# bempt/uda_aerial_semantic_segmentation_research

Measured on AMD Instinct MI355X. Metric: training images/sec at 512x512, higher is better.
Workload: dtype fp32

## Files before the change

include/udaseg.h:

```cpp
#ifndef UDASEG_H
#define UDASEG_H

#include <stddef.h>
#include <stdint.h>

#ifdef __cplusplus
extern "C" {
#endif

#define UDASEG_OK 0
#define UDASEG_E_BADARG (-1)
#define UDASEG_E_UNSUPPORTED (-2)
#define UDASEG_E_WORKSPACE (-3)
#define UDASEG_E_HIP (-4)

#define UDASEG_ACT_NONE 0
#define UDASEG_ACT_LEAKY 1

int udaseg_version(void);
#define UDASEG_OPT_GENERIC_GATHER 0
#define UDASEG_OPT_F32_SPLIT 1
#define UDASEG_OPT_WGRAD_GENERIC 2
#define UDASEG_OPT_F32_HALO 3
#define UDASEG_OPT_F3_CFG 4
#define UDASEG_OPT_F3_WS 5
#define UDASEG_OPT_F3_SIGNS 6
#define UDASEG_OPT_IGEMM_TILE 7
#define UDASEG_OPT_IGEMM_X3 8
#define UDASEG_OPT_NO_FOLD 9
#define UDASEG_OPT_WGRAD_X3_BLOCKS 10
#define UDASEG_OPT_WGRAD_BLOCKS 11
#define UDASEG_OPT_WGRAD_NO_XCD 12
#define UDASEG_OPT_WGRAD_X3 13
#define UDASEG_OPT_NO_WGRAD_HALO 14
#define UDASEG_OPT_WGRAD_F3_BLOCKS 15
#define UDASEG_OPT_WGRAD_HALO_BLOCKS 16
#define UDASEG_OPT_WGRAD_DEEP_BLOCKS 17
#define UDASEG_OPT_WGRAD_DB 18
#define UDASEG_OPT_REDUCE_BLOCKS 19
#define UDASEG_OPT_BN_APPLY_PT 20
#define UDASEG_OPT_GEMM_1X1_TILE 21
#define UDASEG_OPT_GEMM_1X1 22
#define UDASEG_OPT_GEMM_1X1_MAXM 23
#define UDASEG_OPT_NO_STREAM 24
#define UDASEG_OPT_HALO_CFG 25
#define UDASEG_OPT_NO_HALO 26
#define UDASEG_OPT_NO_HALO_S2 27
#define UDASEG_OPT_HALO_W16 28
#define UDASEG_OPT_HALO_DEEP 29
#define UDASEG_OPT_HALO_S2_CK 30
#define UDASEG_OPT_UP_CFG 31
#define UDASEG_OPT_WGRAD_UP_BLOCKS 32
#define UDASEG_OPT_COUNT 33
int udaseg_set_option(int key, int value);
int udaseg_get_option(int key);
int udaseg_option_count(void);
const char* udaseg_option_name(int key);
int udaseg_option_epoch(void);
const char* udaseg_last_error(void);
int udaseg_device_count(void);
int udaseg_memset_async(void* ptr, int value, size_t bytes, void* stream);
int udaseg_stream_wait(void* waiter_stream, void* signal_stream);

typedef struct {
  int n, hi, wi, ci;
  int ho, wo, co;
  int kh, kw, stride, pad;
} udaseg_conv_desc;


int udaseg_conv2d_fwd(const udaseg_conv_desc* d, const float* x, const float* w, const float* bias, float* y,
                      int act, float slope, int accumulate, void* stream);
int udaseg_conv2d_fwd_bnstats(const udaseg_conv_desc* d, const float* x, const float* w, const float* bias, float* y,
                              double* stats, void* stream);
int udaseg_conv2d_fwd_fused(const udaseg_conv_desc* d, const float* x, const float* w, const float* bias,
                            const float* residual, float* y, int act, float slope, void* stream);
int udaseg_conv2d_fwd_bf16(const udaseg_conv_desc* d, const void* x, const void* w, const float* bias, const void* residual,
                           void* y, int out_f32, int act, float slope, double* stats, void* stream);
int udaseg_conv2d_dgrad_bf16(const udaseg_conv_desc* d, const void* dy, const void* w_t, void* dx, int accumulate,
                             void* stream);
int udaseg_conv2d_wgrad_bf16(const udaseg_conv_desc* d, const void* x, const void* dy, float* dw, int accumulate, void* stream);
int udaseg_conv2d_dgrad(const udaseg_conv_desc* d, const float* dy, const float* w_t, float* dx, int accumulate,
                        void* stream);
int udaseg_conv2d_dgrad_bnreduce_ok(const udaseg_conv_desc* d);
int udaseg_conv2d_dgrad_bnreduce(const udaseg_conv_desc* d, const float* dy, const float* w_t, float* dx, const float* prev_y,
                                 const float* save_mean, const float* save_rstd, const float* gamma, const float* beta, int act,
                                 float slope, double* bsums, void* stream);
int udaseg_conv2d_dgrad_bnreduce_bf16_ok(const udaseg_conv_desc* d);
int udaseg_conv2d_dgrad_bnreduce_bf16(const udaseg_conv_desc* d, const void* dy, const void* w_t, void* dx, const void* prev_y,
                                      const float* save_mean, const float* save_rstd, const float* gamma, const float* beta,
                                      int act, float slope, double* bsums, void* stream);
int udaseg_conv2d_wgrad(const udaseg_conv_desc* d, const float* x, const float* dy, float* dw, int accumulate,
                        void* stream);
int udaseg_conv2d_fwd_upcat(const udaseg_conv_desc* d, const float* a, const float* skip, int ca, const float* w,
                            const float* bias, float* y, int act, float slope, double* stats, void* stream);
int udaseg_conv2d_fwd_upcat_bf16(const udaseg_conv_desc* d, const void* a, const void* skip, int ca, const void* w,
                                 const float* bias, void* y, int act, float slope, double* stats, void* stream);
int udaseg_conv2d_dgrad_split(const udaseg_conv_desc* d, const float* dy, const float* w_t, float* dx_a, float* dx_b, int ca,
                              void* stream);
int udaseg_conv2d_dgrad_split_bf16(const udaseg_conv_desc* d, const void* dy, const void* w_t, void* dx_a, void* dx_b, int ca,
                                   void* stream);
int udaseg_conv2d_wgrad_part(const udaseg_conv_desc* d, const float* src, int src_c, int c_off, int up, const float* dy,
                             float* dw, int accumulate, void* stream);
int udaseg_conv2d_wgrad_part_bf16(const udaseg_conv_desc* d, const void* src, int src_c, int c_off, int up, const void* dy,
                                  float* dw, int accumulate, void* stream);
int udaseg_pack_dgrad_weights(const udaseg_conv_desc* d, const float* w, float* w_t, void* stream);
int udaseg_pack_dgrad_batched(const float* arena, float* packed, const int* table, int entries, void* stream);
double udaseg_conv_flops(const udaseg_conv_desc* d);

int udaseg_nchw_to_nhwc(const float* x, float* y, int n, int c, int h, int w, int cpad, void* stream);

int udaseg_bn_replicas(void);
int udaseg_bn_stats(const float* y, int64_t pixels, int c, double* sums, void* stream);
int udaseg_bn_stats_bf16(const void* y, int64_t pixels, int c, double* sums, void* stream);
int udaseg_bn_apply(const float* y, const double* sums, const float* gamma, const float* beta, const float* residual,
                    float* z, int64_t pixels, int c, float eps, float momentum, float* running_mean,
                    float* running_var, float* save_mean, float* save_rstd, int act, float slope, void* stream);
int udaseg_bn_apply_eval(const float* y, const float* gamma, const float* beta, const float* running_mean,
                         const float* running_var, const float* residual, float* z, int64_t pixels, int c, float eps,
                         int act, float slope, void* stream);
int udaseg_bn_fold(const float* w, const float* bias, const float* gamma, const float* beta, const float* running_mean,
                   const float* running_var, float eps, int co, int row_len, float* w_folded, float* bias_folded, void* stream);
int udaseg_bn_bwd_reduce(const float* dz, const float* z, const float* y, const float* save_mean,
                         const float* save_rstd, const float* gamma, const float* beta, int64_t pixels, int c,
                         double* bsums, int act, float slope, void* stream);
int udaseg_bn_bwd_apply(const float* dz, const float* z, const float* y, const float* save_mean,
                        const float* save_rstd, const float* gamma, const float* beta, const double* bsums, float* dy,
                        float* dres, float* dgamma, float* dbeta, int64_t pixels, int c, int act, float slope,
                        int accumulate_dy, int accumulate_dres, int accumulate_param, void* stream);
int udaseg_act_bwd(const float* dz, const float* z, float* dy, int64_t count, int act, float slope, void* stream);
int udaseg_channel_sum(const float* x, int64_t pixels, int c, float* out,
                       int accumulate, void* stream);
int udaseg_channel_sum_ws(const float* x, int64_t pixels, int c, float* out, int accumulate, float* scratch,
                          size_t scratch_bytes, void* stream);
size_t udaseg_channel_sum_scratch_bytes(int c);

// ... 197 lines not shown
```

uda_aerial_semantic_segmentation_research_amd/_lib.py:

```python
import ctypes as C
import os

_HERE = os.path.dirname(os.path.abspath(__file__))
LIB_PATH = os.environ.get("UDASEG_LIB", os.path.join(_HERE, "libudaseg_hip.so"))

ACT_NONE = 0
ACT_LEAKY = 1


class ConvDesc(C.Structure):
    _fields_ = [(k, C.c_int) for k in ("n", "hi", "wi", "ci", "ho", "wo", "co", "kh", "kw", "stride", "pad")]


_P = C.c_void_p
_I = C.c_int
_L = C.c_int64
_F = C.c_float
_D = C.POINTER(ConvDesc)

SIGNATURES = {
    "udaseg_version": (_I, []),
    "udaseg_set_option": (_I, [_I, _I]),
    "udaseg_get_option": (_I, [_I]),
    "udaseg_option_count": (_I, []),
# ... 62 lines not shown
    "udaseg_predict_threshold": (_I, [_P, _I, _I, _I, _I, _P, _P]),
    "udaseg_dice_bwd": (_I, [_P, _P, _P, _P, _F, _I, _L, _I, _I, _P, _I, _P]),
    "udaseg_focal_fwd": (_I, [_P, _P, _P, _F, _F, _L, _I, _I, _I, _P, _P, _I, _P]),
    "udaseg_focal_bwd": (_I, [_P, _P, _P, _F, _F, _P, _F, _L, _I, _I, _P, _I, _P]),
    "udaseg_consistency_fwd": (_I, [_P, _P, _F, _I, _L, _I, _I, _P, _P, _P]),
    "udaseg_consistency_bwd": (_I, [_P, _P, _F, _P, _F, _I, _L, _I, _I, _P, _P, _I, _P]),
    "udaseg_argmax_confusion": (_I, [_P, _P, _L, _I, _I, _P, _P, _P]),
    "udaseg_gap_splits": (_I, [_I]),
    "udaseg_gap_linear_sigmoid_fwd": (_I, [_P, _P, _P, _P, _P, _P, _I, _I, _I, _P]),
    "udaseg_gap_linear_sigmoid_bwd": (_I, [_P, _P, _P, _P, _P, _P, _P, _I, _I, _I, _I, _P]),
    "udaseg_bce_logits_fwd": (_I, [_P, _I, _F, _F, _P, _I, _P]),
    "udaseg_bce_logits_bwd": (_I, [_P, _I, _F, _F, _P, _P, _I, _P]),
    "udaseg_adam_flat": (_I, [_P, _P, _P, _P, _L, _F, _F, _F, _F, _F, _F, _P]),
    "udaseg_bn_apply_bf16": (_I, [_P, _P, _P, _P, _P, _P, _L, _I, _F, _F, _P, _P, _P, _P, _I, _F, _P]),
    "udaseg_bn_bwd_reduce_bf16": (_I, [_P, _P, _P, _P, _P, _L, _I, _P, _I, _F, _P]),
    "udaseg_bn_bwd_apply_bf16": (_I, [_P, _P, _P, _P, _P, _P, _P, _P, _P, _P, _P, _L, _I, _I, _F, _I, _I, _I, _P]),
    "udaseg_act_bwd_bf16": (_I, [_P, _P, _P, _L, _I, _F, _P]),
    "udaseg_channel_sum_bf16": (_I, [_P, _L, _I, _P, _I, _P]),
    "udaseg_channel_sum_bf16_ws": (_I, [_P, _L, _I, _P, _I, _P, C.c_size_t, _P]),
    "udaseg_nchw_to_nhwc_bf16": (_I, [_P, _P, _I, _I, _I, _I, _I, _P]),
    "udaseg_cast_f32_to_bf16": (_I, [_P, _P, _L, _P]),
    "udaseg_maxpool3x3s2_fwd_bf16": (_I, [_P, _P, _P, _I, _I, _I, _I, _P]),
    "udaseg_maxpool3x3s2_bwd_bf16": (_I, [_P, _P, _P, _I, _I, _I, _I, _I, _P]),
    "udaseg_upsample2x_concat_bwd_bf16": (_I, [_P, _P, _P, _I, _I, _I, _I, _I, _I, _I, _P]),
    "udaseg_gap_partial_bf16": (_I, [_P, _P, _I, _I, _I, _P]),
    "udaseg_gap_finish": (_I, [_P, _P, _P, _P, _P, _I, _I, _I, _P]),
    "udaseg_gap_bwd_broadcast_bf16": (_I, [_P, _P, _P, _P, _I, _I, _I, _P]),
    "udaseg_gap_bwd_param": (_I, [_P, _P, _P, _P, _P, _I, _I, _I, _P]),
    "udaseg_pack_dgrad_batched_bf16": (_I, [_P, _P, _P, _I, _P]),
    "udaseg_bn_finalize": (_I, [_P, _P, _P, _L, _I, _F, _F, _P, _P, _P, _P, _P, _P, _P]),
    "udaseg_bn_bwd_apply_recompute_bf16": (_I, [_P, _P, _P, _P, _P, _P, _P, _P, _P, _P, _P, _L, _I, _I, _F, _P]),
    "udaseg_conv2d_wgrad_halo_bf16_ok": (_I, [_D, _I]),
    "udaseg_conv2d_wgrad_halo_bf16": (_I, [_D, _P, _P, _I, _P, _P, _P]),
    "udaseg_conv2d_wgrad_bnin_bf16": (_I, [_D, _P, _P, _P, _I, _F, _P, _P, _I, _P]),
    "udaseg_frag_elems": (_L, [_I, _I, _I]),
    "udaseg_set_stats_scratch": (_I, [_P, C.c_size_t]),
    "udaseg_pack_frag_batched_bf16": (_I, [_P, _P, _P, _P, _I, _P]),
    "udaseg_conv_frag_ok": (_I, [_D, _I, _I]),
    "udaseg_conv_frag_preferred": (_I, [_D, _I, _I]),
    "udaseg_conv2d_fwd_frag_bf16": (_I, [_D, _P, _P, _I, _P, _P, _P, _P, _I, _F, _P, _I, _I, _F, _P, _P]),
    "udaseg_conv2d_dgrad_frag_bf16": (_I, [_D, _P, _P, _P, _P, _I, _P, _P, _P, _P, _P, _I, _F, _P, _I, _P]),
    "udaseg_pack_frag_batched_f32x3": (_I, [_P, _P, _P, _P, _I, _P]),
    "udaseg_conv2d_wgrad_halo_f32x3_ok": (_I, [_D, _I]),
    "udaseg_conv2d_wgrad_halo_f32x3": (_I, [_D, _P, _P, _I, _P, _P, _P]),
    "udaseg_conv_f32x3_ok": (_I, [_D, _I, _I]),
    "udaseg_f32x3_force_config": (_I, [_I]),
    "udaseg_conv_f32x3_preferred": (_I, [_D, _I, _I]),
    "udaseg_conv2d_fwd_f32x3": (_I, [_D, _P, _P, _I, _P, _P, _P, _I, _F, _P, _P]),
    "udaseg_conv2d_fwd_f32x3_bnin_ok": (_I, [_D, _I]),
    "udaseg_conv2d_fwd_f32x3_bnin_writes": (_I, [_D]),
    "udaseg_conv2d_fwd_f32x3_bnin": (_I, [_D, _P, _I, _P, _P, _I, _F, _P, _P, _P, _P, _I, _F, _P, _P]),
    "udaseg_conv2d_wgrad_bnin_ok": (_I, [_D, _I]),
    "udaseg_conv2d_wgrad_bnin": (_I, [_D, _P, _I, _P, _P, _I, _F, _P, _P, _I, _P]),
    "udaseg_conv2d_dgrad_f32x3": (_I, [_D, _P, _P, _P, _P, _I, _P, _P, _P, _P, _P, _I, _F, _P, _I, _P]),
    "udaseg_conv_up_f32x3_ok": (_I, [_D, _I]),
    "udaseg_pack_up_batched_f32x3": (_I, [_P, _P, _P, _P, _I, _P]),
    "udaseg_conv2d_fwd_up_f32x3": (_I, [_D, _P, _I, _P, _P, _I, _P, _P]),
    "udaseg_conv2d_dgrad_up_f32x3": (_I, [_D, _P, _I, _P, _P, _P, _P, _P, _P, _P, _I, _F, _P, _I, _P]),
    "udaseg_up_f32x3_force_config": (_I, [_I]),
    "udaseg_conv2d_wgrad_up_f32x3_ok": (_I, [_D, _I]),
    "udaseg_conv2d_wgrad_up_f32x3": (_I, [_D, _P, _I, _P, _P, _P]),
    "udaseg_conv2d_wgrad_halo_slice_f32x3": (_I, [_D, _P, _P, _P, _I, _I, _P]),
    "udaseg_wgrad_up_set_blocks": (_I, [_I]),
    "udaseg_conv_stem_f32x3_ok": (_I, [_D]),
    "udaseg_conv2d_fwd_stem_f32x3": (_I, [_D, _P, _P, _P, _P, _P]),
    "udaseg_conv_n16_f32x3_ok": (_I, [_D, _I]),
    "udaseg_conv2d_fwd_n16_f32x3": (_I, [_D, _P, _P, _P, _I, _F, _P, _P, _P, _P]),
    "udaseg_conv2d_dgrad_n16_f32x3": (_I, [_D, _P, _P, _P, _P, _P, _P, _P, _P, _I, _F, _P, _P]),
    "udaseg_set_workspace": (_I, [_P, C.c_size_t]),
    "udaseg_workspace_bytes": (C.c_size_t, [_D]),
    "udaseg_debug_set_timeline": (_I, [_P, _I]),
    "udaseg_fill_f32": (_I, [_P, _L, _F, _P]),
    "udaseg_axpy_f32": (_I, [_P, _P, _L, _F, _P]),
    "udaseg_add_i64": (_I, [_P, _L, _L, _P]),
    "udaseg_prof_enable": (_I, [_I]),
    "udaseg_prof_reset": (_I, []),
    "udaseg_prof_read": (_I, [_I, C.POINTER(C.c_double), C.POINTER(C.c_double), C.POINTER(C.c_int64)]),
    "udaseg_prof_kernel_count": (_I, []),
    "udaseg_prof_kernel_name": (C.c_char_p, [_I]),
    "udaseg_prof_kernel_read": (_I, [_I, C.POINTER(C.c_double), C.POINTER(C.c_double), C.POINTER(C.c_int64)]),
    "udaseg_prof_records": (_I, [_I, _I, C.POINTER(C.c_double), C.POINTER(C.c_double), C.POINTER(C.c_int), C.POINTER(C.c_int)]),
}

OPTIONS = {"GENERIC_GATHER": 0, "F32_SPLIT": 1, "WGRAD_GENERIC": 2, "F32_HALO": 3, "F3_CFG": 4, "F3_WS": 5, "F3_SIGNS": 6, "IGEMM_TILE": 7, "IGEMM_X3": 8, "NO_FOLD": 9, "WGRAD_X3_BLOCKS": 10, "WGRAD_BLOCKS": 11, "WGRAD_NO_XCD": 12, "WGRAD_X3": 13, "NO_WGRAD_HALO": 14, "WGRAD_F3_BLOCKS": 15, "WGRAD_HALO_BLOCKS": 16, "WGRAD_DEEP_BLOCKS": 17, "WGRAD_DB": 18, "REDUCE_BLOCKS": 19, "BN_APPLY_PT": 20, "GEMM_1X1_TILE": 21, "GEMM_1X1": 22, "GEMM_1X1_MAXM": 23, "NO_STREAM": 24, "HALO_CFG": 25, "NO_HALO": 26, "NO_HALO_S2": 27, "HALO_W16": 28, "HALO_DEEP": 29, "HALO_S2_CK": 30, "UP_CFG": 31, "WGRAD_UP_BLOCKS": 32}

_lib = None


def load():
    global _lib
    if _lib is not None:
        return _lib
    if not os.path.exists(LIB_PATH):
        raise RuntimeError(
            f"{LIB_PATH} not found: the HIP extension is not built. Run `python -c \"import __graft_entry__ as g; "
            f"g.build()\"` (or `make -C {os.path.join(_HERE, 'csrc')}`). There is no CPU fallback.")
    lib = C.CDLL(LIB_PATH)
    for name, (res, args) in SIGNATURES.items():
        fn = getattr(lib, name)
        fn.restype = res
        fn.argtypes = args
    _lib = lib
    return lib


def check(rc, what=""):
    if rc != 0:
        msg = load().udaseg_last_error().decode(errors="replace")
        raise RuntimeError(f"libudaseg_hip {what} failed (rc={rc}): {msg}")


def require_gpu():
    lib = load()
    if lib.udaseg_device_count() < 1:
        raise RuntimeError("libudaseg_hip: no HIP device visible; this path has no CPU fallback")
    return lib
```

uda_aerial_semantic_segmentation_research_amd/csrc/api.hip:

```cpp
#include <string.h>
#include <mutex>
#include <vector>

#include "common.h"
#include "options.h"

namespace udaseg {

static thread_local char g_err[512] = "";

void set_error(const char* fmt, ...) {
  va_list ap;
  va_start(ap, fmt);
  vsnprintf(g_err, sizeof(g_err), fmt, ap);
  va_end(ap);
}

int hip_fail(hipError_t e, const char* what) {
  set_error("%s: %s", what, hipGetErrorString(e));
  return UDASEG_E_HIP;
}

struct ProfRec {
  hipEvent_t a, b;
// ... 161 lines not shown
    }
    g_krecs[k].clear();
  }
  return UDASEG_OK;
}

extern "C" int udaseg_prof_read(int family, double* total_ms, double* total_flops, int64_t* launches) {
  UDASEG_CHECK_ARG(family >= 0 && family < 2 && total_ms && total_flops && launches, "prof_read: bad arguments");
  double ms = 0.0, fl = 0.0;
  for (auto& r : g_recs[family]) {
    hipError_t e = hipEventSynchronize(r.b);
    if (e != hipSuccess) return hip_fail(e, "hipEventSynchronize(prof)");
    float t = 0.f;
    e = hipEventElapsedTime(&t, r.a, r.b);
    if (e != hipSuccess) return hip_fail(e, "hipEventElapsedTime(prof)");
    ms += t;
    fl += r.flops;
  }
  *total_ms = ms;
  *total_flops = fl;
  *launches = (int64_t)g_recs[family].size();
  return UDASEG_OK;
}

extern "C" int udaseg_prof_records(int family, int max_records, double* ms, double* flops, int* kind, int* desc11) {
  UDASEG_CHECK_ARG(family >= 0 && family < 2 && ms && flops && kind && desc11 && max_records >= 0, "prof_records: bad arguments");
  int n = 0;
  for (auto& r : g_recs[family]) {
    if (n >= max_records) break;
    hipError_t e = hipEventSynchronize(r.b);
    if (e != hipSuccess) return hip_fail(e, "hipEventSynchronize(prof)");
    float t = 0.f;
    e = hipEventElapsedTime(&t, r.a, r.b);
    if (e != hipSuccess) return hip_fail(e, "hipEventElapsedTime(prof)");
    ms[n] = t;
    flops[n] = r.flops;
    kind[n] = r.kind;
    const int v[11] = {r.d.n, r.d.hi, r.d.wi, r.d.ci, r.d.ho, r.d.wo, r.d.co, r.d.kh, r.d.kw, r.d.stride, r.d.pad};
    for (int i = 0; i < 11; ++i) desc11[n * 11 + i] = v[i];
    ++n;
  }
  return n;
}

namespace udaseg {
enum { K_INT, K_FLAG, K_OFF0 };
struct OptRow {
  const char* env;
  int kind, dflt;
};
static const OptRow g_opt_rows[UDASEG_OPT_COUNT] = {
     {"UDASEG_IGEMM_GENERIC", K_INT, 0},
     {"UDASEG_F32_SPLIT", K_OFF0, 1},
     {"UDASEG_WGRAD_GENERIC", K_INT, 0},
     {"UDASEG_F32_SPLIT", K_OFF0, 1},
     {"UDASEG_F3_CFG", K_INT, 0},
     {"UDASEG_F3_WS", K_OFF0, 1},
     {"UDASEG_F3_SIGNS", K_OFF0, 1},
     {"UDASEG_IGEMM_TILE", K_INT, 0},
     {"UDASEG_IGEMM_X3", K_INT, 1},
     {"UDASEG_NO_FOLD", K_FLAG, 0},
     {"UDASEG_WGRAD_X3_BLOCKS", K_INT, 1024},
     {"UDASEG_WGRAD_BLOCKS", K_INT, 0},
     {"UDASEG_WGRAD_NO_XCD", K_FLAG, 0},
     {"UDASEG_WGRAD_X3", K_OFF0, 1},
     {"UDASEG_NO_WGRAD_HALO", K_FLAG, 0},
     {"UDASEG_WGRAD_F3_BLOCKS", K_INT, 120},
     {"UDASEG_WGRAD_HALO_BLOCKS", K_INT, 96},
     {"UDASEG_WGRAD_DEEP_BLOCKS", K_INT, 0},
     {"UDASEG_WGRAD_DB", K_INT, 1},
     {"UDASEG_REDUCE_BLOCKS", K_INT, 0},
     {"UDASEG_BN_APPLY_PT", K_INT, 4},
     {"UDASEG_GEMM_1X1_TILE", K_INT, 0},
     {"UDASEG_GEMM_1X1", K_OFF0, 1},
     {"UDASEG_GEMM_1X1_MAXM", K_INT, 73728},
     {"UDASEG_NO_STREAM", K_FLAG, 0},
     {"UDASEG_HALO_CFG", K_INT, 0},
     {"UDASEG_NO_HALO", K_FLAG, 0},
     {"UDASEG_NO_HALO_S2", K_FLAG, 0},
     {"UDASEG_HALO_W16", K_INT, 6},
     {"UDASEG_HALO_DEEP", K_OFF0, 1},
     {"UDASEG_HALO_S2_CK", K_INT, 64},
     {"UDASEG_UP_CFG", K_INT, 0},
     {"UDASEG_WGRAD_UP_BLOCKS", K_INT, 0}};
int g_opt_val[UDASEG_OPT_COUNT];
static int g_opt_default[UDASEG_OPT_COUNT];
std::atomic<bool> g_opt_ready{false};
static std::atomic<int> g_opt_epoch{0};
static std::mutex g_opt_mutex;
void opt_init() {
  std::lock_guard<std::mutex> lk(g_opt_mutex);
  if (g_opt_ready.load(std::memory_order_relaxed)) return;
  for (int k = 0; k < UDASEG_OPT_COUNT; ++k) {
    const OptRow& r = g_opt_rows[k];
    const char* e = getenv(r.env);
    int v = r.dflt;
    if (r.kind == K_INT) v = e ? atoi(e) : r.dflt;
    else if (r.kind == K_FLAG) v = e != nullptr ? 1 : 0;
    else v = (e && atoi(e) == 0) ? 0 : 1;
    g_opt_default[k] = g_opt_val[k] = v;
  }
  g_opt_ready.store(true, std::memory_order_release);
}
}

extern "C" int udaseg_set_option(int key, int value) {
  UDASEG_CHECK_ARG(key >= 0 && key < UDASEG_OPT_COUNT, "set_option: unknown key %d (0 .. %d)", key, UDASEG_OPT_COUNT - 1);
  UDASEG_CHECK_ARG(value >= -1, "set_option: value must be >= 0, or -1 for the default");
  udaseg::opt_get(key);
  std::lock_guard<std::mutex> lk(udaseg::g_opt_mutex);
  udaseg::g_opt_val[key] = value < 0 ? udaseg::g_opt_default[key] : value;
  if (key == UDASEG_OPT_GENERIC_GATHER)
    udaseg::g_opt_val[UDASEG_OPT_WGRAD_GENERIC] = value < 0 ? udaseg::g_opt_default[UDASEG_OPT_WGRAD_GENERIC] : value;
  udaseg::g_opt_epoch.fetch_add(1);
  return UDASEG_OK;
}

extern "C" int udaseg_get_option(int key) {
  if (key < 0 || key >= UDASEG_OPT_COUNT) return -1;
  return udaseg::opt_get(key);
}

extern "C" int udaseg_option_count(void) { return UDASEG_OPT_COUNT; }
extern "C" const char* udaseg_option_name(int key) { return key >= 0 && key < UDASEG_OPT_COUNT ? udaseg::g_opt_rows[key].env : ""; }
extern "C" int udaseg_option_epoch(void) { return udaseg::g_opt_epoch.load(); }

extern "C" int udaseg_prof_kernel_count(void) { return g_nkernels; }
extern "C" const char* udaseg_prof_kernel_name(int kid) { return kname(kid); }

extern "C" int udaseg_prof_kernel_read(int kid, double* total_ms, double* total_flops, int64_t* launches) {
  UDASEG_CHECK_ARG(kid >= 0 && kid < g_nkernels && total_ms && total_flops && launches, "prof_kernel_read: bad arguments");
  double ms = 0.0, fl = 0.0;
  for (auto& r : g_krecs[kid]) {
    hipError_t e = hipEventSynchronize(r.b);
    if (e != hipSuccess) return hip_fail(e, "hipEventSynchronize(kprof)");
    float t = 0.f;
    e = hipEventElapsedTime(&t, r.a, r.b);
    if (e != hipSuccess) return hip_fail(e, "hipEventElapsedTime(kprof)");
    ms += t;
    fl += r.flops;
  }
  *total_ms = ms;
  *total_flops = fl;
  *launches = (int64_t)g_krecs[kid].size();
  return UDASEG_OK;
}
```

uda_aerial_semantic_segmentation_research_amd/csrc/common.h:

```cpp
#pragma once
#include <stdlib.h>
#include <hip/hip_runtime.h>
#include <stdint.h>
#include <stdio.h>
#include <stdarg.h>
#include <atomic>

#include "../../include/udaseg.h"
#include "options.h"

namespace udaseg {

void set_error(const char* fmt, ...);
int hip_fail(hipError_t e, const char* what);

#define UDASEG_CHECK_ARG(cond, ...)                 \
  do {                                              \
    if (!(cond)) {                                  \
      ::udaseg::set_error(__VA_ARGS__);             \
      return UDASEG_E_BADARG;                       \
    }                                               \
  } while (0)

#define UDASEG_LAUNCH_CHECK(what)                          \
// ... 80 lines not shown
      if (o < co && c < ci) v = *reinterpret_cast<const f32x4*>(w + ((size_t)o * T + t) * ci + c);
#pragma unroll
      for (int k = 0; k < 4; ++k) tile[row][4 * q + k] = v[k];
    }
    __syncthreads();
    {
      const int c = 32 * b + row, o = 32 * a + 4 * q;
      if (c < ci && o < co) {
        OutT* dst = wt + ((size_t)c * T + t) * co + o;
        if constexpr (sizeof(OutT) == 4) {
          f32x4 v;
#pragma unroll
          for (int k = 0; k < 4; ++k) v[k] = tile[4 * q + k][row];
          *reinterpret_cast<f32x4*>(dst) = v;
        } else {
          unsigned short h[4];
#pragma unroll
          for (int k = 0; k < 4; ++k) h[k] = __builtin_bit_cast(unsigned short, (__bf16)tile[4 * q + k][row]);
          uint2 pk;
          pk.x = (unsigned)h[0] | ((unsigned)h[1] << 16);
          pk.y = (unsigned)h[2] | ((unsigned)h[3] << 16);
          *reinterpret_cast<uint2*>(dst) = pk;
        }
      }
    }
    __syncthreads();
  }
}
constexpr int PACK_DGRAD_GRID_X = 256;

void* workspace_ptr(size_t* bytes);

constexpr int CHSUM_REPLICAS = 16;
constexpr int CHSUM_DIRECT_BLOCKS = 32;
static __global__ void fold_replicas_kernel(const float* __restrict__ rep, int c, float* __restrict__ out, int accumulate) {
  const int i = blockIdx.x * blockDim.x + threadIdx.x;
  if (i >= c) return;
  float s = 0.f;
#pragma unroll
  for (int r = 0; r < CHSUM_REPLICAS; ++r) s += rep[(size_t)r * c + i];
  out[i] = accumulate ? out[i] + s : s;
}

struct StreamShape {
  int bs;
  int grid;
  int c4;
};

static inline StreamShape stream_shape(int64_t n4, int c4, int max_blocks = 2048, int per_thread = 4) {
  StreamShape s;
  s.c4 = c4;
  int unit;
  if (c4 <= 256) {
    s.bs = (256 / c4) * c4;
    unit = 1;
  } else {
    s.bs = 256;
    unit = (c4 + 255) / 256;
    while ((unit * 256) % c4 != 0) ++unit;
  }
  int64_t want = (n4 + (int64_t)s.bs * per_thread - 1) / ((int64_t)s.bs * per_thread);
  if (want > max_blocks) want = max_blocks;
  if (want < 1) want = 1;
  s.grid = (int)(((want + unit - 1) / unit) * unit);
  while ((int64_t)s.grid * s.bs < c4) s.grid += unit;
  return s;
}


static inline int apply_per_thread() {
  const int v = opt_get(UDASEG_OPT_BN_APPLY_PT);
  return (v < 1 || v > 256) ? 4 : v;
}

bool small_conv_applicable(int k, int stride, int pad, int ci_gather, int co_out);
int launch_small_conv(const float* x, const float* w, const float* bias, float* y, int n, int h, int wd, int ci, int co,
                      int flip, int accumulate, int act, float slope, double* stats, const float* residual, hipStream_t s,
                      int up = 0);
bool small_wgrad_applicable(int k, int stride, int pad, int ci, int co, int ntiles);
int launch_small_wgrad(const float* x, const float* dy, float* dw, int n, int h, int wd, int ci, int co, int accumulate,
                       hipStream_t s, int up = 0, const float* in_scale = nullptr, const float* in_shift = nullptr,
                       int in_act = 0, float in_slope = 0.f);

constexpr int PROF_NKERNELS = 24;
int kprof_id(const char* rocprof_symbol);
hipEvent_t kprof_begin(hipStream_t s);
void kprof_end(int kid, hipEvent_t a, hipStream_t s, double flops);
struct KTimer {
  std::atomic<int>* kid;
  hipStream_t s;
  hipEvent_t ev;
  double work;
  KTimer(std::atomic<int>* k, const char* rocprof_symbol, hipStream_t st, double w) : kid(k), s(st), work(w) {
    if (*kid < 0) *kid = kprof_id(rocprof_symbol);
    ev = kprof_begin(s);
  }
  ~KTimer() { kprof_end(*kid, ev, s, work); }
};
void prof_begin(int family, hipStream_t s);
void prof_suspend(int on);
void prof_end(int family, hipStream_t s, double flops, int kind, const udaseg_conv_desc* d);

}
```

uda_aerial_semantic_segmentation_research_amd/csrc/conv_small.hip:

```cpp
#include "common.h"

namespace udaseg {

constexpr int ST = 16;
constexpr int SH = ST + 2;

constexpr int MAX_DEVICES = 16;
static void* g_workspace[MAX_DEVICES] = {};
static size_t g_workspace_bytes[MAX_DEVICES] = {};
static int current_device() {
  int dev = 0;
  if (hipGetDevice(&dev) != hipSuccess || dev < 0 || dev >= MAX_DEVICES) return -1;
  return dev;
}

struct SmallArgs {
  const float* x;
  const float* w;
  const float* bias;
  float* y;
  int n, h, wd, ci, co;
  const float* residual;
  double* stats;
  int flip;
// ... 370 lines not shown
__global__ void small_wgrad_fold_kernel(const float* __restrict__ partial, int nblocks, int cop, int cip, int co, int ci,
                                        float* __restrict__ dw) {
  const int out = cop * 9 * cip;
  const int idx = blockIdx.x * blockDim.x + threadIdx.x;
  if (idx >= out) return;
  const int c = idx % cip, t = (idx / cip) % 9, o = idx / (cip * 9);
  if (c >= ci || o >= co) return;
  const int per = (nblocks + gridDim.y - 1) / gridDim.y;
  const int b0 = blockIdx.y * per, b1 = min(nblocks, b0 + per);
  float s[8] = {0.f, 0.f, 0.f, 0.f, 0.f, 0.f, 0.f, 0.f};
  int b = b0;
  for (; b + 8 <= b1; b += 8) {
#pragma unroll
    for (int u = 0; u < 8; ++u) s[u] += partial[(size_t)(b + u) * out + idx];
  }
  for (; b < b1; ++b) s[0] += partial[(size_t)b * out + idx];
  const float tot = ((s[0] + s[1]) + (s[2] + s[3])) + ((s[4] + s[5]) + (s[6] + s[7]));
  if (b1 > b0) atomicAdd(dw + ((size_t)o * 9 + t) * ci + c, tot);
}

static int small_grid(int ntiles, int blocks_per_cu) {
  int g = 256 * blocks_per_cu;
  return ntiles < g ? ntiles : g;
}

bool small_conv_applicable(int k, int stride, int pad, int ci_gather, int co_out) {
  if (k != 3 || stride != 1 || pad != 1) return false;
  const int G = (ci_gather + 15) / 16, T = (co_out + 15) / 16;
  return G * T <= 2;
}

int launch_small_conv(const float* x, const float* w, const float* bias, float* y, int n, int h, int wd, int ci, int co,
                      int flip, int accumulate, int act, float slope, double* stats, const float* residual, hipStream_t s,
                      int up) {
  SmallArgs a = {};
  a.up = up;
  a.x = x; a.w = w; a.bias = bias; a.y = y; a.stats = stats; a.residual = residual;
  a.n = n; a.h = h; a.wd = wd; a.ci = ci; a.co = co;
  a.flip = flip; a.accumulate = accumulate; a.act = act; a.slope = slope;
  a.tiles_x = cdiv(wd, ST); a.tiles_y = cdiv(h, ST); a.ntiles = n * a.tiles_x * a.tiles_y;
  const int G = cdiv(ci, 16), T = cdiv(co, 16);
  dim3 block(256);
  const double fl = 2.0 * (double)n * h * wd * co * 9.0 * ci;
  hipEvent_t ev = kprof_begin(s);
  if (G == 1 && T == 1) {
    hipLaunchKernelGGL((conv3x3_small_kernel<1, 1>), dim3(small_grid(a.ntiles, 6)), block, 0, s, a);
    kprof_end(4, ev, s, fl);
  } else if (G == 2 && T == 1) {
    hipLaunchKernelGGL((conv3x3_small_kernel<2, 1>), dim3(small_grid(a.ntiles, 3)), block, 0, s, a);
    kprof_end(5, ev, s, fl);
  } else if (G == 1 && T == 2) {
    hipLaunchKernelGGL((conv3x3_small_kernel<1, 2>), dim3(small_grid(a.ntiles, 6)), block, 0, s, a);
    kprof_end(6, ev, s, fl);
  } else {
    set_error("small conv: unsupported channel groups G=%d T=%d", G, T);
    return UDASEG_E_UNSUPPORTED;
  }
  UDASEG_LAUNCH_CHECK("conv3x3_small launch");
  return UDASEG_OK;
}

bool small_wgrad_applicable(int k, int stride, int pad, int ci, int co, int ntiles) {
  if (!small_conv_applicable(k, stride, pad, ci, co)) return false;
  const int G = (ci + 15) / 16, T = (co + 15) / 16;
  const size_t need = (size_t)small_grid(ntiles, 2) * (16 * T) * 9 * (16 * G) * sizeof(float);
  const int dev = current_device();
  return dev >= 0 && g_workspace[dev] != nullptr && g_workspace_bytes[dev] >= need;
}

int launch_small_wgrad(const float* x, const float* dy, float* dw, int n, int h, int wd, int ci, int co, int accumulate,
                       hipStream_t s, int up, const float* in_scale, const float* in_shift, int in_act, float in_slope) {
  SmallWgradArgs a = {};
  a.up = up;
  a.in_scale = in_scale; a.in_shift = in_shift; a.in_act = in_act; a.in_slope = in_slope;
  const int dev = current_device();
  if (dev < 0 || g_workspace[dev] == nullptr) {
    set_error("small wgrad: no workspace bound to the current device");
    return UDASEG_E_WORKSPACE;
  }
  a.x = x; a.dy = dy; a.partial = static_cast<float*>(g_workspace[dev]);
  a.n = n; a.h = h; a.w = wd; a.ci = ci; a.co = co;
  a.tiles_x = cdiv(wd, ST); a.tiles_y = cdiv(h, ST); a.ntiles = n * a.tiles_x * a.tiles_y;
  const int G = cdiv(ci, 16), T = cdiv(co, 16);
  const int grid = small_grid(a.ntiles, 2);
  dim3 block(256);
  const double fl = 2.0 * (double)n * h * wd * co * 9.0 * ci;
  hipEvent_t ev = kprof_begin(s);
  if (G == 1 && T == 1) {
    hipLaunchKernelGGL((conv3x3_small_wgrad_kernel<1, 1>), dim3(grid), block, 0, s, a);
    kprof_end(9, ev, s, fl);
  } else if (G == 2 && T == 1) {
    hipLaunchKernelGGL((conv3x3_small_wgrad_kernel<2, 1>), dim3(grid), block, 0, s, a);
    kprof_end(10, ev, s, fl);
  } else if (G == 1 && T == 2) {
    hipLaunchKernelGGL((conv3x3_small_wgrad_kernel<1, 2>), dim3(grid), block, 0, s, a);
    kprof_end(11, ev, s, fl);
  } else {
    set_error("small wgrad: unsupported channel groups G=%d T=%d", G, T);
    return UDASEG_E_UNSUPPORTED;
  }
  UDASEG_LAUNCH_CHECK("conv3x3_small_wgrad launch");
  const int out = 16 * T * 9 * 16 * G;
  if (!accumulate) {
    hipError_t e = hipMemsetAsync(dw, 0, (size_t)co * 9 * ci * sizeof(float), s);
    if (e != hipSuccess) return hip_fail(e, "hipMemsetAsync(small wgrad)");
  }
  hipLaunchKernelGGL(small_wgrad_fold_kernel, dim3(cdiv(out, 256), FOLD_SLICES), dim3(256), 0, s, a.partial, grid, 16 * T, 16 * G,
                     co, ci, dw);
  UDASEG_LAUNCH_CHECK("small_wgrad_fold launch");
  return UDASEG_OK;
}

}

namespace udaseg {
void* workspace_ptr(size_t* bytes) {
  const int dev = current_device();
  if (dev < 0 || g_workspace[dev] == nullptr) {
    if (bytes) *bytes = 0;
    return nullptr;
  }
  if (bytes) *bytes = g_workspace_bytes[dev];
  return g_workspace[dev];
}
}

extern "C" size_t udaseg_workspace_bytes(const udaseg_conv_desc* d) {
  if (!d || d->kh != d->kw || !udaseg::small_conv_applicable(d->kh, d->stride, d->pad, d->ci, d->co)) return 0;
  const int G = (d->ci + 15) / 16, T = (d->co + 15) / 16;
  const int ntiles = d->n * udaseg::cdiv(d->hi, udaseg::ST) * udaseg::cdiv(d->wi, udaseg::ST);
  return (size_t)udaseg::small_grid(ntiles, 2) * (16 * T) * 9 * (16 * G) * sizeof(float);
}

extern "C" int udaseg_set_workspace(void* ptr, size_t bytes) {
  const int dev = udaseg::current_device();
  UDASEG_CHECK_ARG(dev >= 0, "set_workspace: no current HIP device (or more than %d devices)", udaseg::MAX_DEVICES);
  udaseg::g_workspace[dev] = ptr;
  udaseg::g_workspace_bytes[dev] = ptr ? bytes : 0;
  return UDASEG_OK;
}
```

Before: 1111.

## Add bf16x3 MFMA weight-gradient kernel for small-channel 3x3 convolutions

Adds a new weight-gradient kernel for small-channel (16/32) 3x3 convs that splits fp32 inputs into three bf16 pieces and accumulates with bf16 MFMA, replacing the previous small wgrad path when the option and f32 halo mode are on. It uses LDS transposed reads, prefetches the next tile into registers, and reduces per-block partials through the existing fold kernel. The workspace size is enlarged to hold the x3 kernel's grid of partials. The aim is to move these wgrads off slower scalar/fp32 math onto matrix cores, with some risk of precision drift from the 3-term split and extra LDS pressure.

```diff
diff --git a/include/udaseg.h b/include/udaseg.h
--- a/include/udaseg.h
+++ b/include/udaseg.h
@@ -51,7 +51,8 @@
 #define UDASEG_OPT_HALO_S2_CK 30
 #define UDASEG_OPT_UP_CFG 31
 #define UDASEG_OPT_WGRAD_UP_BLOCKS 32
-#define UDASEG_OPT_COUNT 33
+#define UDASEG_OPT_SMALL_WGRAD_X3 33
+#define UDASEG_OPT_COUNT 34
 int udaseg_set_option(int key, int value);
 int udaseg_get_option(int key);
 int udaseg_option_count(void);
diff --git a/uda_aerial_semantic_segmentation_research_amd/_lib.py b/uda_aerial_semantic_segmentation_research_amd/_lib.py
--- a/uda_aerial_semantic_segmentation_research_amd/_lib.py
+++ b/uda_aerial_semantic_segmentation_research_amd/_lib.py
@@ -168,7 +168,7 @@
     "udaseg_prof_records": (_I, [_I, _I, C.POINTER(C.c_double), C.POINTER(C.c_double), C.POINTER(C.c_int), C.POINTER(C.c_int)]),
 }
 
-OPTIONS = {"GENERIC_GATHER": 0, "F32_SPLIT": 1, "WGRAD_GENERIC": 2, "F32_HALO": 3, "F3_CFG": 4, "F3_WS": 5, "F3_SIGNS": 6, "IGEMM_TILE": 7, "IGEMM_X3": 8, "NO_FOLD": 9, "WGRAD_X3_BLOCKS": 10, "WGRAD_BLOCKS": 11, "WGRAD_NO_XCD": 12, "WGRAD_X3": 13, "NO_WGRAD_HALO": 14, "WGRAD_F3_BLOCKS": 15, "WGRAD_HALO_BLOCKS": 16, "WGRAD_DEEP_BLOCKS": 17, "WGRAD_DB": 18, "REDUCE_BLOCKS": 19, "BN_APPLY_PT": 20, "GEMM_1X1_TILE": 21, "GEMM_1X1": 22, "GEMM_1X1_MAXM": 23, "NO_STREAM": 24, "HALO_CFG": 25, "NO_HALO": 26, "NO_HALO_S2": 27, "HALO_W16": 28, "HALO_DEEP": 29, "HALO_S2_CK": 30, "UP_CFG": 31, "WGRAD_UP_BLOCKS": 32}
+OPTIONS = {"GENERIC_GATHER": 0, "F32_SPLIT": 1, "WGRAD_GENERIC": 2, "F32_HALO": 3, "F3_CFG": 4, "F3_WS": 5, "F3_SIGNS": 6, "IGEMM_TILE": 7, "IGEMM_X3": 8, "NO_FOLD": 9, "WGRAD_X3_BLOCKS": 10, "WGRAD_BLOCKS": 11, "WGRAD_NO_XCD": 12, "WGRAD_X3": 13, "NO_WGRAD_HALO": 14, "WGRAD_F3_BLOCKS": 15, "WGRAD_HALO_BLOCKS": 16, "WGRAD_DEEP_BLOCKS": 17, "WGRAD_DB": 18, "REDUCE_BLOCKS": 19, "BN_APPLY_PT": 20, "GEMM_1X1_TILE": 21, "GEMM_1X1": 22, "GEMM_1X1_MAXM": 23, "NO_STREAM": 24, "HALO_CFG": 25, "NO_HALO": 26, "NO_HALO_S2": 27, "HALO_W16": 28, "HALO_DEEP": 29, "HALO_S2_CK": 30, "UP_CFG": 31, "WGRAD_UP_BLOCKS": 32, "SMALL_WGRAD_X3": 33}
 
 _lib = None
 
diff --git a/uda_aerial_semantic_segmentation_research_amd/csrc/api.hip b/uda_aerial_semantic_segmentation_research_amd/csrc/api.hip
--- a/uda_aerial_semantic_segmentation_research_amd/csrc/api.hip
+++ b/uda_aerial_semantic_segmentation_research_amd/csrc/api.hip
@@ -267,7 +267,8 @@
      {"UDASEG_HALO_DEEP", K_OFF0, 1},
      {"UDASEG_HALO_S2_CK", K_INT, 64},
      {"UDASEG_UP_CFG", K_INT, 0},
-     {"UDASEG_WGRAD_UP_BLOCKS", K_INT, 0}};
+     {"UDASEG_WGRAD_UP_BLOCKS", K_INT, 0},
+     {"UDASEG_SMALL_WGRAD_X3", K_OFF0, 1}};
 int g_opt_val[UDASEG_OPT_COUNT];
 static int g_opt_default[UDASEG_OPT_COUNT];
 std::atomic<bool> g_opt_ready{false};
diff --git a/uda_aerial_semantic_segmentation_research_amd/csrc/common.h b/uda_aerial_semantic_segmentation_research_amd/csrc/common.h
--- a/uda_aerial_semantic_segmentation_research_amd/csrc/common.h
+++ b/uda_aerial_semantic_segmentation_research_amd/csrc/common.h
@@ -186,6 +186,10 @@
 int launch_small_wgrad(const float* x, const float* dy, float* dw, int n, int h, int wd, int ci, int co, int accumulate,
                        hipStream_t s, int up = 0, const float* in_scale = nullptr, const float* in_shift = nullptr,
                        int in_act = 0, float in_slope = 0.f);
+bool small_wgrad_x3_on();
+int small_wgrad_x3_blocks(int n, int h, int wd, int ci, int co);
+int launch_small_wgrad_x3(const float* x, const float* dy, float* partial, int n, int h, int wd, int ci, int co, int up,
+                          const float* in_scale, const float* in_shift, int in_act, float in_slope, int* grid, hipStream_t s);
 
 constexpr int PROF_NKERNELS = 24;
 int kprof_id(const char* rocprof_symbol);
diff --git a/uda_aerial_semantic_segmentation_research_amd/csrc/conv_small.hip b/uda_aerial_semantic_segmentation_research_amd/csrc/conv_small.hip
--- a/uda_aerial_semantic_segmentation_research_amd/csrc/conv_small.hip
+++ b/uda_aerial_semantic_segmentation_research_amd/csrc/conv_small.hip
@@ -476,24 +476,36 @@
   a.n = n; a.h = h; a.w = wd; a.ci = ci; a.co = co;
   a.tiles_x = cdiv(wd, ST); a.tiles_y = cdiv(h, ST); a.ntiles = n * a.tiles_x * a.tiles_y;
   const int G = cdiv(ci, 16), T = cdiv(co, 16);
-  const int grid = small_grid(a.ntiles, 2);
+  int grid = small_grid(a.ntiles, 2);
   dim3 block(256);
   const double fl = 2.0 * (double)n * h * wd * co * 9.0 * ci;
-  hipEvent_t ev = kprof_begin(s);
-  if (G == 1 && T == 1) {
+  int rc = UDASEG_E_UNSUPPORTED;
+  if (small_wgrad_x3_on()) {
+    int cap = (int)(g_workspace_bytes[dev] / ((size_t)16 * T * 9 * 16 * G * sizeof(float)));
+    rc = launch_small_wgrad_x3(x, dy, a.partial, n, h, wd, ci, co, up, in_scale, in_shift, in_act, in_slope, &cap, s);
+    if (rc == UDASEG_OK) grid = cap;
+  }
+  if (rc != UDASEG_E_UNSUPPORTED) {
+    if (rc != UDASEG_OK) return rc;
+  } else if (G == 1 && T == 1) {
+    hipEvent_t ev = kprof_begin(s);
     hipLaunchKernelGGL((conv3x3_small_wgrad_kernel<1, 1>), dim3(grid), block, 0, s, a);
     kprof_end(9, ev, s, fl);
+    UDASEG_LAUNCH_CHECK("conv3x3_small_wgrad launch");
   } else if (G == 2 && T == 1) {
+    hipEvent_t ev = kprof_begin(s);
     hipLaunchKernelGGL((conv3x3_small_wgrad_kernel<2, 1>), dim3(grid), block, 0, s, a);
     kprof_end(10, ev, s, fl);
+    UDASEG_LAUNCH_CHECK("conv3x3_small_wgrad launch");
   } else if (G == 1 && T == 2) {
+    hipEvent_t ev = kprof_begin(s);
     hipLaunchKernelGGL((conv3x3_small_wgrad_kernel<1, 2>), dim3(grid), block, 0, s, a);
     kprof_end(11, ev, s, fl);
+    UDASEG_LAUNCH_CHECK("conv3x3_small_wgrad launch");
   } else {
     set_error("small wgrad: unsupported channel groups G=%d T=%d", G, T);
     return UDASEG_E_UNSUPPORTED;
   }
-  UDASEG_LAUNCH_CHECK("conv3x3_small_wgrad launch");
   const int out = 16 * T * 9 * 16 * G;
   if (!accumulate) {
     hipError_t e = hipMemsetAsync(dw, 0, (size_t)co * 9 * ci * sizeof(float), s);
@@ -523,7 +535,12 @@
   if (!d || d->kh != d->kw || !udaseg::small_conv_applicable(d->kh, d->stride, d->pad, d->ci, d->co)) return 0;
   const int G = (d->ci + 15) / 16, T = (d->co + 15) / 16;
   const int ntiles = d->n * udaseg::cdiv(d->hi, udaseg::ST) * udaseg::cdiv(d->wi, udaseg::ST);
-  return (size_t)udaseg::small_grid(ntiles, 2) * (16 * T) * 9 * (16 * G) * sizeof(float);
+  int blocks = udaseg::small_grid(ntiles, 2);
+  if (G * T <= 2) {
+    const int b3 = udaseg::small_wgrad_x3_blocks(d->n, d->hi, d->wi, d->ci, d->co);
+    if (b3 > blocks) blocks = b3;
+  }
+  return (size_t)blocks * (16 * T) * 9 * (16 * G) * sizeof(float);
 }
 
 extern "C" int udaseg_set_workspace(void* ptr, size_t bytes) {
diff --git a/uda_aerial_semantic_segmentation_research_amd/csrc/conv_small_wgrad_f32x3.hip b/uda_aerial_semantic_segmentation_research_amd/csrc/conv_small_wgrad_f32x3.hip
--- /dev/null
+++ b/uda_aerial_semantic_segmentation_research_amd/csrc/conv_small_wgrad_f32x3.hip
@@ -0,0 +1,311 @@
+#include "common.h"
+#include "halo_common.h"
+
+namespace udaseg {
+
+typedef short sw3_s16x4 __attribute__((ext_vector_type(4)));
+typedef short sw3_s16x8 __attribute__((ext_vector_type(8)));
+
+struct SmallWgradX3Args {
+  const float* x;
+  const float* dy;
+  float* partial;
+  int n, h, w, ci, co, up;
+  int ntx, nty, ntiles;
+  unsigned x_bytes, dy_bytes;
+  int signs;
+  const float* in_scale;
+  const float* in_shift;
+  int in_act;
+  float in_slope;
+};
+
+template <int G, int T>
+struct SW3 {
+  static constexpr int TR = 4, TW = 32, HR = TR + 2, HW = TW + 2, RW = TR / 4;
+  static constexpr int HPX = HR * HW, TPX = TR * TW;
+  static constexpr int CIP = 16 * G, COP = 16 * T;
+  static constexpr int XSP = HPX * 32;
+  static constexpr int DSP = TPX * 32 + 128;
+  static constexpr int XPL = G * XSP, DPL = T * DSP;
+  static constexpr int LDS = 3 * (XPL + DPL);
+  static constexpr int OUT = COP * 9 * CIP;
+  static constexpr int XO = CIP / 8, DO = COP / 8;
+  static constexpr int XPC = HPX * XO, DPC = TPX * DO;
+  static constexpr int NX = (XPC + 255) / 256, ND = (DPC + 255) / 256;
+  static_assert(LDS <= 160 * 1024 && OUT * 4 <= LDS, "LDS");
+  static_assert(256 % XO == 0, "one channel octet per staging thread");
+  static constexpr int WPE = G * T == 1 ? 3 : 2;
+};
+
+__device__ __forceinline__ bf16x8 sw3_fragment(const char* p) {
+  const sw3_s16x4 lo = __builtin_amdgcn_ds_read_tr16_b64_v4i16((sw3_s16x4 __attribute__((address_space(3)))*)(p));
+  const sw3_s16x4 hi = __builtin_amdgcn_ds_read_tr16_b64_v4i16((sw3_s16x4 __attribute__((address_space(3)))*)(p + 512));
+  const sw3_s16x8 f = __builtin_shufflevector(lo, hi, 0, 1, 2, 3, 4, 5, 6, 7);
+  return __builtin_bit_cast(bf16x8, f);
+}
+
+template <int G, int T>
+__global__ __launch_bounds__(256) __attribute__((amdgpu_waves_per_eu(SW3<G, T>::WPE))) void conv3x3_small_wgrad_x3_kernel(
+    const SmallWgradX3Args a) {
+  using C = SW3<G, T>;
+  extern __shared__ __attribute__((aligned(16))) char sw3smem[];
+  char* const Xs = sw3smem;
+  char* const Ds = sw3smem + 3 * C::XPL;
+  const int tid = threadIdx.x, lane = tid & 63;
+  const int wave = __builtin_amdgcn_readfirstlane(tid >> 6);
+  const int H = a.h, W = a.w;
+
+  __amdgpu_buffer_rsrc_t rs_x = __builtin_amdgcn_make_buffer_rsrc(const_cast<float*>(a.x), 0, (int)a.x_bytes, 0x00020000);
+  __amdgpu_buffer_rsrc_t rs_d = __builtin_amdgcn_make_buffer_rsrc(const_cast<float*>(a.dy), 0, (int)a.dy_bytes, 0x00020000);
+  const int xoct = tid % C::XO;
+  const bool xf = a.in_scale != nullptr;
+  f32x4 xsc[2], xsh[2];
+#pragma unroll
+  for (int l = 0; l < 2; ++l) {
+    const int c = 8 * xoct + 4 * l;
+    xsc[l] = xsh[l] = f32x4{0.f, 0.f, 0.f, 0.f};
+    if (xf && c < a.ci) {
+      xsc[l] = *reinterpret_cast<const f32x4*>(a.in_scale + c);
+      xsh[l] = *reinterpret_cast<const f32x4*>(a.in_shift + c);
+    }
+  }
+  u32x4 sx[C::NX][2], sd[C::ND][2];
+  unsigned x_in = 0;
+  auto load_tile = [&](int tile) {
+    const int tx = tile % a.ntx, t2 = tile / a.ntx;
+    const int ty = t2 % a.nty, img = t2 / a.nty;
+    const int y0 = ty * C::TR, x0 = tx * C::TW;
+    x_in = 0;
+#pragma unroll
+    for (int i = 0; i < C::NX; ++i) {
+      const int pc = tid + 256 * i;
+      const int pix = pc / C::XO;
+      const int hy = pix / C::HW, hx = pix - hy * C::HW;
+      const int iy = y0 + hy - 1, ix = x0 + hx - 1;
+      const bool ok = pc < C::XPC && (unsigned)iy < (unsigned)H && (unsigned)ix < (unsigned)W;
+      const int p = a.up ? (img * (H >> 1) + (iy >> 1)) * (W >> 1) + (ix >> 1) : (img * H + iy) * W + ix;
+#pragma unroll
+      for (int l = 0; l < 2; ++l) {
+        const int c = 8 * xoct + 4 * l;
+        const bool in = ok && c < a.ci;
+        x_in |= (in ? 1u : 0u) << (2 * i + l);
+        const unsigned off = in ? (unsigned)(p * a.ci + c) * 4u : 0x80000000u;
+        sx[i][l] = __builtin_amdgcn_raw_buffer_load_b128(rs_x, (int)off, 0, 0);
+      }
+    }
+#pragma unroll
+    for (int i = 0; i < C::ND; ++i) {
+      const int pc = tid + 256 * i;
+      const int pix = pc / C::DO, oct = pc % C::DO;
+      const int oy = y0 + pix / C::TW, ox = x0 + pix % C::TW;
+      const bool ok = pc < C::DPC && oy < H && ox < W;
+      const int p = (img * H + oy) * W + ox;
+#pragma unroll
+      for (int l = 0; l < 2; ++l) {
+        const int c = 8 * oct + 4 * l;
+        const unsigned off = ok && c < a.co ? (unsigned)(p * a.co + c) * 4u : 0x80000000u;
+        sd[i][l] = __builtin_amdgcn_raw_buffer_load_b128(rs_d, (int)off, 0, 0);
+      }
+    }
+  };
+  auto store_piece = [&](char* dst, int plane_bytes, const u32x4& lo, const u32x4& hi) {
+    u32x4 p0, p1, p2;
+    split3(lo, hi, p0, p1, p2);
+    *reinterpret_cast<u32x4*>(dst) = p0;
+    *reinterpret_cast<u32x4*>(dst + plane_bytes) = p1;
+    *reinterpret_cast<u32x4*>(dst + 2 * plane_bytes) = p2;
+  };
+  auto store_tile = [&](bool neg) {
+#pragma unroll
+    for (int i = 0; i < C::NX; ++i) {
+      const int pc = tid + 256 * i;
+      const int pix = pc / C::XO;
+      if (xf) {
+#pragma unroll
+        for (int l = 0; l < 2; ++l) {
+          const bool in = (x_in >> (2 * i + l)) & 1u;
+          f32x4 v = __builtin_bit_cast(f32x4, sx[i][l]);
+#pragma unroll
+          for (int e = 0; e < 4; ++e) {
+            const float t = act_apply(__builtin_fmaf(v[e], xsc[l][e], xsh[l][e]), a.in_act, a.in_slope);
+            v[e] = in ? t : 0.f;
+          }
+          sx[i][l] = __builtin_bit_cast(u32x4, v);
+        }
+      }
+      if (i < C::NX - 1 || pc < C::XPC) store_piece(Xs + (xoct >> 1) * C::XSP + pix * 32 + (xoct & 1) * 16, C::XPL, sx[i][0], sx[i][1]);
+    }
+    const unsigned sgn = neg ? 0x80000000u : 0u;
+#pragma unroll
+    for (int i = 0; i < C::ND; ++i) {
+      const int pc = tid + 256 * i;
+      const int pix = pc / C::DO, oct = pc % C::DO;
+      if (i < C::ND - 1 || pc < C::DPC)
+        store_piece(Ds + (oct >> 1) * C::DSP + pix * 32 + (oct & 1) * 16, C::DPL, sd[i][0] ^ sgn, sd[i][1] ^ sgn);
+    }
+  };
+
+  f32x4 acc[3][3][G][T];
+#pragma unroll
+  for (int r = 0; r < 3; ++r)
+#pragma unroll
+    for (int s = 0; s < 3; ++s)
+#pragma unroll
+      for (int g = 0; g < G; ++g)
+#pragma unroll
+        for (int t = 0; t < T; ++t) acc[r][s][g][t] = f32x4{0.f, 0.f, 0.f, 0.f};
+
+  const int gq = lane >> 4, q = (lane >> 2) & 3, pp = lane & 3;
+  const int lane_off = (4 * gq + q) * 32 + pp * 8;
+  const int r0 = C::RW * wave;
+  const char* const dbase = Ds + r0 * C::TW * 32 + lane_off;
+  const char* const xbase = Xs + r0 * C::HW * 32 + lane_off;
+
+  const int nseq = (int)blockIdx.x < a.ntiles ? (a.ntiles - (int)blockIdx.x + (int)gridDim.x - 1) / (int)gridDim.x : 0;
+  const int sq1 = a.signs ? (nseq + 2) / 4 : 0, sq3 = a.signs ? nseq - sq1 : 0;
+  bool negated = false;
+  int seq = 0;
+  if (nseq > 0) load_tile(blockIdx.x);
+  for (int tile = blockIdx.x; tile < a.ntiles; tile += gridDim.x, ++seq) {
+    const bool neg = seq >= sq1 && seq < sq3;
+    __syncthreads();
+    store_tile(neg);
+    __syncthreads();
+    if (tile + (int)gridDim.x < a.ntiles) load_tile(tile + gridDim.x);
+    if (neg != negated) {
+      negated = neg;
+#pragma unroll
+      for (int r = 0; r < 3; ++r)
+#pragma unroll
+        for (int s = 0; s < 3; ++s)
+#pragma unroll
+          for (int g = 0; g < G; ++g)
+#pragma unroll
+            for (int t = 0; t < T; ++t) acc[r][s][g][t] = -acc[r][s][g][t];
+    }
+    bf16x8 A[C::RW][T][3];
+#pragma unroll
+    for (int rr = 0; rr < C::RW + 2; ++rr) {
+      if (rr < C::RW) {
+#pragma unroll
+        for (int t = 0; t < T; ++t)
+#pragma unroll
+          for (int pl = 0; pl < 3; ++pl) A[rr][t][pl] = sw3_fragment(dbase + pl * C::DPL + t * C::DSP + rr * C::TW * 32);
+      }
+#pragma unroll
+      for (int g = 0; g < G; ++g) {
+        bf16x8 B[3][3];
+#pragma unroll
+        for (int s = 0; s < 3; ++s)
+#pragma unroll
+          for (int pl = 0; pl < 3; ++pl) B[s][pl] = sw3_fragment(xbase + pl * C::XPL + g * C::XSP + (rr * C::HW + s) * 32);
+#pragma unroll
+        for (int r = 0; r < 3; ++r) {
+          const int j = rr - r;
+          if (j >= 0 && j < C::RW) {
+#pragma unroll
+            for (int s = 0; s < 3; ++s)
+#pragma unroll
+              for (int t = 0; t < T; ++t)
+#pragma unroll
+                for (int ij = 2; ij >= 0; --ij)
+#pragma unroll
+                  for (int i = 0; i <= ij; ++i)
+                    acc[r][s][g][t] = __builtin_amdgcn_mfma_f32_16x16x32_bf16(A[j][t][i], B[s][ij - i], acc[r][s][g][t], 0, 0, 0);
+          }
+        }
+      }
+    }
+  }
+  if (negated) {
+#pragma unroll
+    for (int r = 0; r < 3; ++r)
+#pragma unroll
+      for (int s = 0; s < 3; ++s)
+#pragma unroll
+        for (int g = 0; g < G; ++g)
+#pragma unroll
+          for (int t = 0; t < T; ++t) acc[r][s][g][t] = -acc[r][s][g][t];
+  }
+
+  float* const red = reinterpret_cast<float*>(sw3smem);
+  const int li = lane & 15;
+  __syncthreads();
+  for (int wv = 0; wv < 4; ++wv) {
+    if (wave == wv) {
+#pragma unroll
+      for (int r = 0; r < 3; ++r)
+#pragma unroll
+        for (int s = 0; s < 3; ++s)
+#pragma unroll
+          for (int g = 0; g < G; ++g)
+#pragma unroll
+            for (int t = 0; t < T; ++t)
+#pragma unroll
+              for (int v = 0; v < 4; ++v) {
+                const int idx = ((16 * t + 4 * gq + v) * 9 + 3 * r + s) * C::CIP + 16 * g + li;
+                red[idx] = (wv == 0 ? 0.f : red[idx]) + acc[r][s][g][t][v];
+              }
+    }
+    __syncthreads();
+  }
+  float* dst = a.partial + (size_t)blockIdx.x * C::OUT;
+  for (int idx = tid; idx < C::OUT; idx += 256) dst[idx] = red[idx];
+}
+
+template <int G, int T>
+static int launch_sw3_t(const SmallWgradX3Args& a, int cap, int* grid, hipStream_t s, double flops) {
+  using C = SW3<G, T>;
+  auto kern = conv3x3_small_wgrad_x3_kernel<G, T>;
+  const int g = cap < small_wgrad_x3_blocks(a.n, a.h, a.w, a.ci, a.co) ? cap : small_wgrad_x3_blocks(a.n, a.h, a.w, a.ci, a.co);
+  *grid = g;
+  static std::atomic<bool> attr_done{false};
+  if (!attr_done) {
+    hipError_t e = hipFuncSetAttribute(reinterpret_cast<const void*>(kern), hipFuncAttributeMaxDynamicSharedMemorySize, C::LDS);
+    if (e != hipSuccess) return hip_fail(e, "hipFuncSetAttribute(conv3x3_small_wgrad_x3)");
+    attr_done = true;
+  }
+  static std::atomic<int> kid{-1};
+  if (kid < 0) {
+    char nm[64];
+    snprintf(nm, sizeof(nm), "conv3x3_small_wgrad_x3_kernel<%d, %d>", G, T);
+    kid = kprof_id(nm);
+  }
+  hipEvent_t ev = kprof_begin(s);
+  hipLaunchKernelGGL(kern, dim3(g), dim3(256), C::LDS, s, a);
+  kprof_end(kid, ev, s, flops);
+  UDASEG_LAUNCH_CHECK("conv3x3_small_wgrad_x3 launch");
+  return UDASEG_OK;
+}
+
+int small_wgrad_x3_blocks(int n, int h, int wd, int ci, int co) {
+  const int ntiles = n * cdiv(h, SW3<1, 1>::TR) * cdiv(wd, SW3<1, 1>::TW);
+  const int g = 256 * (cdiv(ci, 16) * cdiv(co, 16) == 1 ? SW3<1, 1>::WPE : SW3<2, 1>::WPE);
+  return ntiles < g ? ntiles : g;
+}
+
+bool small_wgrad_x3_on() {
+  return opt_get(UDASEG_OPT_SMALL_WGRAD_X3) != 0 && f32_halo_enabled();
+}
+
+int launch_small_wgrad_x3(const float* x, const float* dy, float* partial, int n, int h, int wd, int ci, int co, int up,
+                          const float* in_scale, const float* in_shift, int in_act, float in_slope, int* grid, hipStream_t s) {
+  const int G = cdiv(ci, 16), T = cdiv(co, 16);
+  const long long xb = (long long)n * (up ? (h >> 1) * (wd >> 1) : h * wd) * ci * 4, db = (long long)n * h * wd * co * 4;
+  if (xb >= (1LL << 31) || db >= (1LL << 31) || !(G * T == 1 || (G == 2 && T == 1) || (G == 1 && T == 2))) return UDASEG_E_UNSUPPORTED;
+  SmallWgradX3Args a = {};
+  a.x = x; a.dy = dy; a.partial = partial;
+  a.n = n; a.h = h; a.w = wd; a.ci = ci; a.co = co; a.up = up;
+  a.ntx = cdiv(wd, SW3<1, 1>::TW); a.nty = cdiv(h, SW3<1, 1>::TR); a.ntiles = n * a.ntx * a.nty;
+  a.x_bytes = (unsigned)xb; a.dy_bytes = (unsigned)db;
+  a.signs = f3_signs_on() ? 1 : 0;
+  a.in_scale = in_scale; a.in_shift = in_shift; a.in_act = in_act; a.in_slope = in_slope;
+  const double fl = 2.0 * (double)n * h * wd * co * 9.0 * ci;
+  const int cap = *grid;
+  if (G == 1 && T == 1) return launch_sw3_t<1, 1>(a, cap, grid, s, fl);
+  if (G == 2) return launch_sw3_t<2, 1>(a, cap, grid, s, fl);
+  return launch_sw3_t<1, 2>(a, cap, grid, s, fl);
+}
+
+}
```

After: 1118, median of 6. Within noise of the previous version (+0.7%).
